# tgsstdio/BirdNest.Audio

Hardware: AMD Instinct MI355X
Metric: decoded PCM MSamples/s/GPU (bit-exact) + achieved HBM GB/s vs roofline (higher is better)
Workload: dtype int32; 1 GPU; C2: 1024-frame batches, 44.1 kHz/16-bit stereo, bs 4096, LPC-8, Rice partition order 4 -> FLACDecoder 16-bit LE interleaved PCM; frames_per_batch=1024, compressed_bytes_per_batch=10724000, pcm_bytes_per_batch=16777216, parallelism=corpus of 1 x 1024 batches partitioned per rank (shard.partition) x1

## Files before the change

birdnest/audio_amd/csrc/bnflac_kernels.hip:

```cpp
#include <hip/hip_runtime.h>
#include <stdint.h>
#include <stdlib.h>
#include <atomic>
#include <mutex>
#include <type_traits>

#include "bnflac_device.h"

#define DEV __device__ __forceinline__

__constant__ uint8_t g_crc8_tab[256];
__constant__ uint16_t g_crc16_tab[8][256];
__constant__ uint16_t g_crc16_xpow[40];
__device__ unsigned long long g_stats[16];
DEV uint64_t tnow(bool on) {
#ifndef BNFLAC_PHASE_TIMERS
    (void)on;
    return 0ull;
#endif
    if (!on) return 0ull;
    const uint64_t t = __builtin_amdgcn_s_memtime();
    asm volatile("s_waitcnt lgkmcnt(0)" ::: "memory");
    return t;
}
// ... 9 lines not shown
}
DEV u32x4 lds_ld128(const void *a) {
    u32x4 v;
    asm volatile("ds_read_b128 %0, %1" : "=v"(v) : "v"((uint32_t)(uintptr_t)a) : "memory");
    return v;
}
DEV void lds_st128(const lds_u32x4 *a, u32x4 v) {
    asm volatile("ds_write_b128 %0, %1" ::"v"((uint32_t)(uintptr_t)a), "v"(v) : "memory");
}
DEV u32x4 lds_ld128(const lds_u32x4 *a) {
    u32x4 v;
    asm volatile("ds_read_b128 %0, %1" : "=v"(v) : "v"((uint32_t)(uintptr_t)a) : "memory");
    return v;
}
DEV void lds_st64(const void *a, uint64_t v) {
    asm volatile("ds_write_b64 %0, %1" ::"v"((uint32_t)(uintptr_t)a), "v"(v) : "memory");
}
DEV uint64_t lds_ld64(const void *a) {
    uint64_t v;
    asm volatile("ds_read_b64 %0, %1" : "=v"(v) : "v"((uint32_t)(uintptr_t)a) : "memory");
    return v;
}
typedef __attribute__((address_space(1))) const void gvoid;
DEV void gst128(uint64_t addr, u32x4 v) { *(__attribute__((address_space(1))) u32x4 *)addr = v; }

#define BNF_MODE_WREDO 0x4000u
#define BNF_MODE_SW 0x8000u
#define BNF_ABLATE_NO_SW 0x10000u
#define BNF_MODE_LIST 0x20000u
#define BNF_MODE_SEG 0x80000000u
#define BNF_MODE_NOST 0x40000u
#define BNF_MODE_STREDO 0x80000u
#define BNF_ABLATE_NO_W8SPLIT 0x100000u

#define RING_MAX 16
#define RING_LANE_DW 256

struct BR {
    const uint32_t *__restrict__ w;
    uint32_t nw;
    uint32_t nblk;
    lds_u32 *ring;
    lds_u32 *lring;
    uint32_t rdepth, wmask;
    uint32_t wi, s, hi, lo, nx;
    uint32_t vendw, iend;
    uint32_t iend_old;
    uint32_t ra, vlim;
    bool stats;
};

DEV void br_init(BR &b, const uint32_t *words, uint64_t nbytes, lds_u32 *ring, uint32_t lane, uint32_t rdepth) {
    b.rdepth = rdepth;
    b.wmask = 4u * rdepth - 1u;
    b.w = words;
    b.nblk = (uint32_t)((nbytes + 15u) >> 4);
    b.nw = b.nblk * 4u;
    b.ring = ring;
    b.lring = ring + lane * 4u;
    b.wi = 2;
    b.s = b.hi = b.lo = b.nx = 0;
    b.vendw = b.iend = 0;
    b.iend_old = 0;
    b.stats = false;
}

// ... 614 lines not shown
#define CRC_LINES 4

DEV uint32_t byte_keep(int32_t lo, int32_t hi, int32_t w) {
    const int32_t a = min(max(lo - 4 * w, 0), 4), b = min(max(hi - 4 * w, 0), 4);
    const uint32_t mlo = a >= 4 ? 0u : (0xFFFFFFFFu << (8 * a));
    const uint32_t mhi = b >= 4 ? 0xFFFFFFFFu : ((1u << (8 * b)) - 1u);
    return mlo & mhi;
}
DEV bool crcz_zero(const CrcZ &c) {
    if (__builtin_popcount(c.px) & 1) return false;
    uint64_t v = ((uint64_t)(c.r1 & 0x0FFFFFFFu) << 32) | c.r0;
#pragma unroll
    for (int i = 0; i < 4; i++) {
        const uint64_t h = v >> 15;
        v = (v & 0x7FFFu) ^ h ^ (h << 1);
    }
    return v == 0;
}
DEV void crcz_line(CrcZ &c, uint4 (&v)[4], uint32_t h) {
    if (h) {
#pragma unroll
        for (int u = 0; u < 4; u++) {
            v[u].x &= st_hmask(h, 16u * u);
            v[u].y &= st_hmask(h, 16u * u + 4u);
            v[u].z &= st_hmask(h, 16u * u + 8u);
            v[u].w &= st_hmask(h, 16u * u + 12u);
        }
    }
#pragma unroll
    for (int u = 0; u < 4; u++) crcz_blk(c, v[u]);
}
template <int NL = CRC_LINES>
DEV bool st_crc16_ok(const uint8_t *__restrict__ bytes, uint64_t b0, uint64_t b1, CrcZ c = CrcZ{0u, 0u, 0u},
                     uint64_t from = 0) {
    const uint64_t p0 = max(b0 & ~(uint64_t)63u, from);
    const uint32_t h = p0 < b0 ? (uint32_t)(b0 & 63u) : 0u;
    const uint32_t nl = b1 > p0 ? (uint32_t)((b1 - p0) >> 6) : 0u;
    uint64_t p = p0;
    if (nl) {
        const uint4 *q = (const uint4 *)(bytes + p0);
        uint4 buf[NL][4];
#pragma unroll
        for (int d = 0; d < NL; d++)
#pragma unroll
            for (int u = 0; u < 4; u++) buf[d][u] = q[4u * min((uint32_t)d, nl - 1u) + u];
#pragma unroll
        for (int u = 0; u < 4; u++) {
            buf[0][u].x &= st_hmask(h, 16u * u);
            buf[0][u].y &= st_hmask(h, 16u * u + 4u);
            buf[0][u].z &= st_hmask(h, 16u * u + 8u);
            buf[0][u].w &= st_hmask(h, 16u * u + 12u);
        }
        for (uint32_t i = 0; i < nl; i += NL) {
#pragma unroll
            for (int d = 0; d < NL; d++) {
                if (i + d < nl) {
#pragma unroll
                    for (int u = 0; u < 4; u++) crcz_blk(c, buf[d][u]);
                    const uint32_t j = min(i + d + NL, nl - 1u);
#pragma unroll
                    for (int u = 0; u < 4; u++) buf[d][u] = q[4u * j + u];
                }
            }
        }
        p = p0 + (uint64_t)nl * 64u;
    }
    const uint32_t nr = (uint32_t)((b1 - p + 15u) >> 4);
    uint4 t[4];
#pragma unroll
    for (uint32_t i = 0; i < 4; i++) t[i] = i < nr ? *(const uint4 *)(bytes + p + 16u * i) : make_uint4(0u, 0u, 0u, 0u);
#pragma unroll
    for (uint32_t i = 0; i < 4; i++) {
        if (i < nr) {
            const int64_t lo = (int64_t)b0 - (int64_t)(p + 16u * i), hi = (int64_t)b1 - (int64_t)(p + 16u * i);
            const int32_t l32 = (int32_t)max(min(lo, (int64_t)16), (int64_t)0);
            const int32_t h32 = (int32_t)max(min(hi, (int64_t)16), (int64_t)0);
            uint4 v = t[i];
            v.x &= byte_keep(l32, h32, 0);
            v.y &= byte_keep(l32, h32, 1);
            v.z &= byte_keep(l32, h32, 2);
            v.w &= byte_keep(l32, h32, 3);
            crcz_blk(c, v);
        }
    }
    return crcz_zero(c);
}
#define CRCP_WORDS 8u
DEV bool st_crc16_frame(const uint8_t *__restrict__ bytes, const uint32_t *__restrict__ crcp, uint32_t f, uint64_t b0,
                        uint64_t b1) {
    if (crcp) {
        const u32x4 v = *(const u32x4 *)(crcp + CRCP_WORDS * (uint64_t)f + 4u);
        if (v.x && v.z == (uint32_t)b0 && b0 + v.x == b1) return v.y != 0u;
        const u32x4 q = *(const u32x4 *)(crcp + CRCP_WORDS * (uint64_t)f);
        const uint64_t from = ((b0 >> 6) + q.z - 1u) * 64u;
        if (q.z && q.w == (uint32_t)b0 && from <= b1)
            return st_crc16_ok(bytes, b0, b1, CrcZ{q.x, q.y & 0x0FFFFFFFu, q.y >> 31}, from);
    }
    return st_crc16_ok(bytes, b0, b1);
}

DEV uint32_t ffbh_b(uint32_t x) { return x ? (uint32_t)__builtin_clz(x) : ~0u; }

DEV uint32_t pk_ra(uint32_t wi, uint32_t lane) { return ((wi & 3u) << 2) | (lane << 4) | (((wi >> 2) & 7u) << 10); }
DEV void pk_resync(BR &b, uint32_t lane) {
    b.ra = pk_ra(b.wi, lane);
    b.vlim = b.vendw - 1u;
}
DEV void pk_next_word(BR &b) { b.nx = *(const lds_u32 *)((const __attribute__((address_space(3))) uint8_t *)b.ring + b.ra); }
DEV void pk_step(BR &b, uint32_t &rem, uint32_t k1, bool &stall, uint32_t laneb) {
    const bool live = rem != 0u;
    const uint32_t w = br_peek(b);
    const uint32_t q1 = min(ffbh_b(w), 32u);
    const uint32_t len1 = q1 + k1;
    const uint32_t q2 = ffbh_b((w << (len1 & 31u)) | 1u);
    const uint32_t len2 = len1 + q2 + k1;
    const bool fit1 = live & (len1 <= 32u);
    const bool fit2 = fit1 & (rem >= 2u) & (len2 <= 32u);
// ... 1859 lines not shown
                                                    uint64_t *__restrict__ d_offs, uint64_t *__restrict__ d_os,
                                                    bnf_frame_info *__restrict__ d_info, uint32_t cap,
                                                    uint32_t *__restrict__ nframes) {
    const uint32_t i = blockIdx.x * 256u + threadIdx.x;
    if (i >= ncand || !mark[i]) return;
    const uint32_t p = pos[i];
    if (p >= cap) return;
    const uint64_t os = out_sample[p];
    if (sp.has_stream_info && sp.total_samples > 0 && os >= sp.total_samples) {
        atomicMin(nframes, p);
        return;
    }
    d_offs[p] = cand[i];
    if (d_os) d_os[p] = os;
    if (d_info) {
        bnf_frame_info fi = info[i];
        fi.out_sample = os;
        d_info[p] = fi;
    }
}
#endif

#if BNF_TU == 3 || BNF_TU == 4 || BNF_TU == 7
#define ST_CHK 16
#define ST2_CHK 32
#define ST_RD 8

struct StCh {
    BR b;
    uint32_t cp[4];
    uint32_t q[8];
    int32_t sh;
    uint32_t k, km, k1, k32;
    uint32_t esc, left, pidx, nparts, psamples, plen, pesc, porder, order;
    uint32_t wasted;
    int32_t lim, mx, mn;
};

DEV uint32_t st_pk(int32_t lo, int32_t hi) { return __builtin_amdgcn_perm((uint32_t)hi, (uint32_t)lo, 0x05040100u); }
typedef short st_s2 __attribute__((ext_vector_type(2)));
DEV int32_t st_d2(uint32_t a, uint32_t b, int32_t acc) {
    return __builtin_amdgcn_sdot2(__builtin_bit_cast(st_s2, a), __builtin_bit_cast(st_s2, b), acc, false);
}
DEV int32_t st_d2z(uint32_t a, uint32_t b) {
    int32_t r;
    asm("v_dot2_i32_i16 %0, %1, %2, 0" : "=v"(r) : "v"(a), "v"(b));
    return r;
}

DEV bool st_setup(StCh &z, uint32_t bps, uint32_t bs, uint64_t limit) {
    SubHdr h;
    int32_t warm[8], coef[8], err = -1;
    const uint32_t st = parse_subframe_head<true, 8>(z.b, bps, bs, limit, h, warm, coef, err);
    if (st != BNF_ST_OK) return false;
    if (h.type != T_FIXED && h.type != T_LPC) return false;
    if (h.type == T_LPC && (h.order > 8 || h.path == P_WIDE)) return false;
    if (h.bps > 17) return false;
    int32_t c[8], w[8];
    bool in16 = true;
#pragma unroll
    for (int t = 0; t < 8; t++) {
        c[t] = 0;
        w[t] = ((uint32_t)t < h.order) ? warm[t] : 0;
        in16 = in16 && w[t] >= -32768 && w[t] <= 32767;
    }
    if (!in16) return false;
    z.sh = 0;
    z.lim = 0x7FFF;
    if (h.type == T_LPC) {
#pragma unroll
        for (int t = 0; t < 8; t++) c[t] = ((uint32_t)t < h.order) ? coef[t] : 0;
        if (h.path == P_MMX16) z.sh = ((uint32_t)h.shift >= 32u) ? 31 : h.shift;
        else z.sh = h.shift & 31;
    } else {
        const uint32_t o = h.order;
        c[0] = o == 1 ? 1 : o == 2 ? 2 : o == 3 ? 3 : o == 4 ? 4 : 0;
        c[1] = o == 2 ? -1 : o == 3 ? -3 : o == 4 ? -6 : 0;
        c[2] = o == 3 ? 1 : o == 4 ? 4 : 0;
        c[3] = o == 4 ? -1 : 0;
    }
#pragma unroll
    for (int k = 0; k < 4; k++) z.cp[k] = st_pk(c[2 * k], c[2 * k + 1]);
#pragma unroll
    for (int t = 0; t < 8; t++) z.q[t] = st_pk(w[t], t ? w[t - 1] : 0);
    z.order = h.order;
    z.wasted = h.wasted;
    z.porder = h.porder;
    z.nparts = 1u << h.porder;
    z.psamples = h.porder ? bs >> h.porder : bs - h.order;
    z.plen = h.rice2 ? 5u : 4u;
    z.pesc = h.rice2 ? 31u : 15u;
    z.left = 0;
    z.pidx = 0;
    z.esc = 0;
    z.k = 0;
    z.km = 31;
    z.k1 = 1;
    z.k32 = 32;
    z.mx = 0;
    z.mn = 0;
    return true;
}

template <class Z>
DEV void st_partition(Z &z) {
    const uint32_t kk = br_read(z.b, z.plen);
    z.left = (z.porder == 0 || z.pidx > 0) ? z.psamples : z.psamples - z.order;
    if (kk < z.pesc) {
        z.k = kk;
        z.esc = 0;
    } else {
        z.k = br_read(z.b, 5);
        z.esc = 1;
    }
    z.km = 31u - z.k;
    z.k1 = z.k + 1u;
    z.k32 = 32u - z.k;
    z.pidx++;
}

DEV void st_land(BR &b, uint32_t nst) {
    STAT(b.stats, 2);
    wait_vm_n(nst);
    b.vendw = b.iend * 4u;
    if (b.wi >= b.vendw) {
        br_refill(b);
        wait_vm();
// ... 16 lines not shown

template <class Z>
DEV int32_t st_rice(Z &z, uint64_t limit, uint32_t &trunc, uint32_t nst) {
    const uint32_t w = br_peek(z.b);
    const uint32_t q = ffbh(w);
    const bool slow = q >= z.k32;
    uint32_t u = (q << z.k) | __builtin_amdgcn_ubfe(w, z.km - q, z.k);
    const bool anyslow = any_lane(slow);
    st_adv(z.b, slow ? 0u : q + z.k1, nst);
    if (__builtin_expect(anyslow, 0)) {
        STAT(z.b.stats, 3);
        if (slow) {
            uint32_t qq;
            if (!br_unary(z.b, qq, limit)) trunc = 1;
            u = (qq << z.k) | br_read(z.b, z.k);
        }
    }
    return (int32_t)((u >> 1) ^ (0u - (u & 1u)));
}

template <class Z>
DEV int32_t st_next(Z &z, uint64_t limit, uint32_t &trunc, uint32_t nst) {
    while (z.left == 0) {
        if (z.pidx >= z.nparts) {
            trunc = 1;
            return 0;
        }
        st_partition(z);
    }
    z.left--;
    if (z.esc) return br_read_s(z.b, z.k);
    return st_rice(z, limit, trunc, nst);
}

template <int I>
DEV void st_dot2(const StCh &a, const StCh &b, int32_t &pa, int32_t &pb) {
#define Q_(z, j) z.q[(I + 8 - (j)) & 7]
    pa = st_d2(a.cp[3], Q_(a, 7), st_d2(a.cp[2], Q_(a, 5), st_d2(a.cp[1], Q_(a, 3), st_d2z(a.cp[0], Q_(a, 1)))));
    pb = st_d2(b.cp[3], Q_(b, 7), st_d2(b.cp[2], Q_(b, 5), st_d2(b.cp[1], Q_(b, 3), st_d2z(b.cp[0], Q_(b, 1)))));
#undef Q_
}

template <int T>
DEV void st_pre2(const StCh &a, const StCh &b, int32_t &pa, int32_t &pb) {
#define P_(z, j) z.q[(T + 8 - (j)) & 7]
    pa = st_d2(a.cp[3], P_(a, 6), st_d2(a.cp[2], P_(a, 4), st_d2z(a.cp[1], P_(a, 2))));
    pb = st_d2(b.cp[3], P_(b, 6), st_d2(b.cp[2], P_(b, 4), st_d2z(b.cp[1], P_(b, 2))));
#undef P_
}
DEV void st_fin2(const StCh &a, const StCh &b, uint32_t qa, uint32_t qb, int32_t prea, int32_t preb, int32_t &pa,
                 int32_t &pb) {
    pa = st_d2(a.cp[0], qa, prea);
    pb = st_d2(b.cp[0], qb, preb);
}

DEV void st_range(StCh &z, int32_t s0, int32_t s1) {
    z.mx = max(z.mx, max(s0, s1));
    z.mn = min(z.mn, min(s0, s1));
}

DEV void st_decor4(bool uni, uint32_t as_u, uint32_t as, int32_t (&L)[4], int32_t (&R)[4]) {
    const uint32_t a = uni ? as_u : as;
    if (a == 1) {
#pragma unroll
        for (int q = 0; q < 4; q++) R[q] = (int32_t)((uint32_t)L[q] - (uint32_t)R[q]);
    } else if (a == 2) {
// ... 84 lines not shown
        }
    }
    return true;
}

DEV uint32_t st_refill_issue(BR &b, bool want) {
    const uint32_t cg = (b.wi >> 2) & ~3u;
    const bool go = want && b.iend == cg + 4u;
    const uint32_t h = b.iend & 4u;
    const bool whole = b.iend + 3u < b.nblk;
    const uint32_t *a = b.w + (uint64_t)b.iend * 4u;
    uint32_t nd = 0;
#pragma unroll
    for (int g = 0; g < 2; g++) {
        const bool gg = go && h == 4u * (uint32_t)g;
        if (__any(gg)) {
            nd += 4u;
            if (gg) {
                lds_u32 *row = b.ring + 4u * (uint32_t)g * RING_LANE_DW;
                if (__builtin_expect(whole, 1)) {
                    lds_dma16_off<0>(a, row);
                    lds_dma16_off<16>(a, row + RING_LANE_DW);
                    lds_dma16_off<32>(a, row + 2 * RING_LANE_DW);
                    lds_dma16_off<48>(a, row + 3 * RING_LANE_DW);
                } else {
#pragma unroll
                    for (int k = 0; k < 4; k++) dma_block(b, b.iend + (uint32_t)k, 4u * (uint32_t)g + (uint32_t)k);
                }
            }
        }
    }
    if (go) b.iend += 4u;
    return nd;
}


DEV uint32_t st_ra(uint32_t wi, uint32_t lane) { return ((wi & 3u) << 2) | (lane << 4) | (((wi >> 2) & 7u) << 10); }
DEV void st_adv_nc(BR &b, uint32_t n, uint32_t laneb) {
    uint32_t t;
    const bool c = __builtin_usub_overflow(b.s, n, &t);
    b.s = t & 31u;
    b.hi = c ? b.lo : b.hi;
    b.lo = c ? __builtin_bswap32(b.nx) : b.lo;
    b.wi += (uint32_t)c;
    b.ra = (((b.ra | 0x3F3u) + (uint32_t)c) & 0x1C0Cu) | laneb;
}
DEV void st_next_word(BR &b) { b.nx = *(const lds_u32 *)((const __attribute__((address_space(3))) uint8_t *)b.ring + b.ra); }
DEV void st_resync(BR &b, uint32_t lane) {
    b.ra = st_ra(b.wi, lane);
    b.vlim = b.vendw - 1u;
}
template <class Z>
DEV void st_rare(Z &z, bool sl, bool ld, uint32_t &u, uint64_t limit, uint32_t &trunc, uint32_t nst,
                uint32_t lane) {
    if (any_lane(ld)) {
        st_land(z.b, nst);
        if (z.b.wi + 1u >= z.b.vendw) {
            wait_vm();
            br_refill(z.b);
            wait_vm();
            br_drained(z.b);
        }
        st_next_word(z.b);
    }
    if (any_lane(sl)) {
        STAT(z.b.stats, 3);
// ... 30 lines not shown
    switch (i) {
    case 0: lo = st_qperm<0x00>(lo); hi = st_qperm<0x00>(hi); break;
    case 1: lo = st_qperm<0x55>(lo); hi = st_qperm<0x55>(hi); break;
    case 2: lo = st_qperm<0xAA>(lo); hi = st_qperm<0xAA>(hi); break;
    default: lo = st_qperm<0xFF>(lo); hi = st_qperm<0xFF>(hi); break;
    }
    return ((uint64_t)hi << 32) | lo;
}

template <int T, int FMT, int AS, int PO, int NPK>
DEV void st_lpc_out(StCh &z0, StCh &z1, uint32_t u0, uint32_t u1, int32_t (&L)[4], int32_t (&R)[4], bool as_uni,
                    uint32_t as_u, uint32_t as, uint8_t *dst, uint32_t nbase, bool al, uint32_t bs, bool store,
                    u32x4 (&pk)[NPK], int32_t &pre0, int32_t &pre1, bool anyw) {
    constexpr bool STG = (FMT == BNF_OUT_FLACDECODER || FMT == BNF_OUT_FILEREADER);
    int32_t p0, p1, n0, n1;
    st_fin2(z0, z1, z0.q[(T + 7) & 7], z1.q[(T + 7) & 7], pre0, pre1, p0, p1);
    st_pre2<T>(z0, z1, n0, n1);
    pre0 = n0;
    pre1 = n1;
    const int32_t s0 = (int32_t)(((u0 >> 1) ^ (0u - (u0 & 1u))) + (uint32_t)(p0 >> z0.sh));
    const int32_t s1 = (int32_t)(((u1 >> 1) ^ (0u - (u1 & 1u))) + (uint32_t)(p1 >> z1.sh));
    if (T & 1) {
        st_range(z0, L[(T + 3) & 3], s0);
        st_range(z1, R[(T + 3) & 3], s1);
    }
    z0.q[T] = __builtin_amdgcn_perm(z0.q[(T + 7) & 7], (uint32_t)s0, 0x05040100u);
    z1.q[T] = __builtin_amdgcn_perm(z1.q[(T + 7) & 7], (uint32_t)s1, 0x05040100u);
    L[T & 3] = s0;
    R[T & 3] = s1;
    if ((T & 3) == 3) {
        if (AS < 0 && __builtin_expect(anyw, 0)) {
#pragma unroll
            for (int q = 0; q < 4; q++) {
                L[q] = (int32_t)((uint32_t)L[q] << z0.wasted);
                R[q] = (int32_t)((uint32_t)R[q] << z1.wasted);
            }
        }
        if (STG && AS >= 0) {
            pk[PO + (T >> 2)] = st_pack4<AS>(z0.q[(T + 6) & 7], z1.q[(T + 6) & 7], z0.q[T], z1.q[T]);
            return;
        }
        st_decor4t<AS>(as_uni, as_u, as, L, R);
        if (STG) {
            uint32_t w[4];
#pragma unroll
            for (int q = 0; q < 4; q++) w[q] = __builtin_amdgcn_perm((uint32_t)R[q], (uint32_t)L[q], 0x05040100u);
            pk[PO + (T >> 2)] = u32x4{w[0], w[1], w[2], w[3]};
        } else if (store) {
            st_emit4<FMT>(dst, nbase + (uint32_t)T - 3u, 4u, al, bs, L, R);
        }
    }
}

DEV uint32_t st_rice_pair(const StCh &z, uint32_t &ua, uint32_t &ub, bool &sl) {
    const uint32_t w = br_peek(z.b);
    const uint32_t qa = (uint32_t)__builtin_clz(w | 1u);
    const uint32_t la = qa + z.k1;
    const uint32_t w2 = w << (la & 31u);
    const uint32_t qb = (uint32_t)__builtin_clz(w2 | 1u);
    ua = (qa << z.k) | __builtin_amdgcn_ubfe(w, z.km - qa, z.k);
    ub = (qb << z.k) | __builtin_amdgcn_ubfe(w2, z.km - qb, z.k);
    const uint32_t n = la + qb + z.k1;
    sl = n > 32u;
    return sl ? 0u : n;
}
DEV void st_rare_pair(StCh &z, bool sl, bool ld, uint32_t &ua, uint32_t &ub, uint64_t limit, uint32_t &trunc,
                      uint32_t nst, uint32_t lane) {
    if (any_lane(ld)) {
// ... 24 lines not shown
                       uint32_t bs, bool store, u32x4 (&pk)[NPK], int32_t &pre0, int32_t &pre1,
                       uint32_t lane, bool anyw) {
    static_assert((T & 1) == 0, "pairs start on even samples");
    constexpr bool STG = (FMT == BNF_OUT_FLACDECODER || FMT == BNF_OUT_FILEREADER);
    constexpr uint32_t spg = (FMT == BNF_OUT_INTERLEAVED32 || FMT == BNF_OUT_PLANAR32) ? 2u : 1u;
    const uint32_t nqt = nq + ((!STG && T >= 4 && store) ? spg : 0u);
    uint32_t u0a, u0b, u1a, u1b;
    bool sl0, sl1;
    const uint32_t n0 = st_rice_pair(z0, u0a, u0b, sl0), n1 = st_rice_pair(z1, u1a, u1b, sl1);
    const uint32_t laneb = lane << 4;
    st_adv_nc(z0.b, n0, laneb);
    st_adv_nc(z1.b, n1, laneb);
    constexpr bool CHK = (T & 2) == 0;
    const bool ld0 = CHK && z0.b.wi >= z0.b.vlim, ld1 = CHK && z1.b.wi >= z1.b.vlim;
    st_next_word(z0.b);
    st_next_word(z1.b);
    if (__builtin_expect(any_lane(sl0 || sl1 || ld0 || ld1), 0)) {
        st_rare_pair(z0, sl0, ld0, u0a, u0b, limit, trunc, nqt, lane);
        st_rare_pair(z1, sl1, ld1, u1a, u1b, limit, trunc, nqt, lane);
    }
    st_lpc_out<T, FMT, AS, PO, NPK>(z0, z1, u0a, u1a, L, R, as_uni, as_u, as, dst, nbase, al, bs, store, pk, pre0, pre1, anyw);
    st_lpc_out<T + 1, FMT, AS, PO, NPK>(z0, z1, u0b, u1b, L, R, as_uni, as_u, as, dst, nbase, al, bs, store, pk, pre0, pre1, anyw);
}

template <int T, int FMT>
DEV bool st_gen_step(StCh &z0, StCh &z1, int32_t (&L)[4], int32_t (&R)[4], uint64_t limit, uint32_t &trunc,
                     uint32_t nst, bool as_uni, uint32_t as_u, uint32_t as, uint8_t *dst, uint32_t n, bool valid,
                     bool al, uint32_t bs, bool store) {
    const bool v = valid && n < bs;
    int32_t s0 = 0, s1 = 0;
    if (v) {
        int32_t p0, p1;
        st_dot2<T>(z0, z1, p0, p1);
        if (n < z0.order) s0 = (int32_t)(int16_t)z0.q[T];
        else s0 = (int32_t)((uint32_t)st_next(z0, limit, trunc, nst) + (uint32_t)(p0 >> z0.sh));
        if (n < z1.order) s1 = (int32_t)(int16_t)z1.q[T];
        else s1 = (int32_t)((uint32_t)st_next(z1, limit, trunc, nst) + (uint32_t)(p1 >> z1.sh));
        st_range(z0, s0, s0);
        st_range(z1, s1, s1);
        z0.q[T] = __builtin_amdgcn_perm(z0.q[(T + 7) & 7], (uint32_t)s0, 0x05040100u);
        z1.q[T] = __builtin_amdgcn_perm(z1.q[(T + 7) & 7], (uint32_t)s1, 0x05040100u);
    }
    L[T & 3] = (int32_t)((uint32_t)s0 << z0.wasted);
    R[T & 3] = (int32_t)((uint32_t)s1 << z1.wasted);
    bool stored = false;
    if ((T & 3) == 3) {
        const uint32_t nq = n - 3u;
        const uint32_t nv = (valid && nq < bs) ? min(4u, bs - nq) : 0u;
        st_decor4(as_uni, as_u, as, L, R);
        if (store) stored = st_emit4<FMT>(dst, nq, nv, al, bs, L, R);
    }
    return stored;
}

template <int FMT>
__global__ void __launch_bounds__(64, 2) k_decode_st(const uint32_t *__restrict__ words, uint64_t nbytes,
                                                     uint32_t nframes, bnf_stream_params sp, uint32_t chn_lanes,
                                                     uint8_t *__restrict__ out, uint64_t out_bytes,
                                                     bnf_frame_info *__restrict__ info,
                                                     const uint32_t *__restrict__ perm, uint32_t ablate,
                                                     const uint32_t *__restrict__ crcp) {
    constexpr bool STG = (FMT == BNF_OUT_FLACDECODER || FMT == BNF_OUT_FILEREADER);
    constexpr uint32_t ST_SPG = (FMT == BNF_OUT_INTERLEAVED32 || FMT == BNF_OUT_PLANAR32) ? 2u : 1u;
    __shared__ LDS_DMA_ALIGN uint32_t ring[2 * ST_RD * RING_LANE_DW + 1024];
    static_assert((ST_RD * RING_LANE_DW * 4) % 1024 == 0, "channel 1's ring base must stay 1 KiB aligned (LDS-DMA)");
    const uint32_t lane = threadIdx.x;
    const uint32_t slot = blockIdx.x * 64u + lane;
    const uint32_t f = (perm && slot < nframes) ? perm[slot] : slot;
    const uint64_t limit = nbytes * 8u;
    bnf_frame_info fi;
    const bool have = f < nframes;
    if (have) fi = info[f];
    const bool mine = have && fi.status == BNF_ST_OK && (fi.flags & BNF_FL_ST) && !(fi.flags & BNF_FL_REDO) &&
                      (!(ablate & BNF_MODE_WREDO) || (fi.flags & BNF_FL_WAVE_REDO));
    if (!__any(mine)) return;

    uint64_t stride = 0;
    bool ok = mine && fi.channels == 2 && chn_lanes >= 2;
    if (FMT == BNF_OUT_FLACDECODER) { stride = 4; ok = ok && fi.bps == 16 && sp.channels >= 2; }
    else if (FMT == BNF_OUT_FILEREADER) { stride = 4; ok = ok && sp.channels == 2 && sp.bps == 16; }
    else if (FMT == BNF_OUT_INTERLEAVED32) { stride = 8; ok = ok && sp.channels == 2; }
    else { stride = 4ull * sp.channels; ok = ok && sp.channels == 2; }
    const uint32_t bs = ok ? fi.blocksize : 0u;
    const uint64_t os = ok ? fi.out_sample : 0u;
    ok = ok && (os + bs) * stride <= out_bytes;
    uint8_t *dst = out + os * stride;
    const bool al = (((uintptr_t)dst) & 15u) == 0 && (FMT != BNF_OUT_PLANAR32 || (bs & 3u) == 0);

    StCh z0, z1;
    lds_u32 *ring0 = (lds_u32 *)ring, *ring1 = (lds_u32 *)ring + ST_RD * RING_LANE_DW;
    br_init(z0.b, words, nbytes, ring0, lane, ST_RD);
    br_init(z1.b, words, nbytes, ring1, lane, ST_RD);
    z0.b.stats = z1.b.stats = (ablate & 0x100u) != 0;
    STAT(z0.b.stats, 5);
    const bool tmon = z0.b.stats;
    const uint64_t t_start = tnow(tmon);
    uint64_t tm_dec = 0, tm_ref = 0, tm_pack = 0;
    if (ok) {
        br_seek(z0.b, fi.frame_off * 8u + fi.sub_start[0]);
        ok = st_setup(z0, sub_bps(fi, 0), bs, limit);
    }
    if (ok) {
        br_seek(z1.b, fi.frame_off * 8u + fi.sub_start[1]);
        ok = st_setup(z1, sub_bps(fi, 1), bs, limit);
    }
    const uint32_t as = ok ? fi.assignment : 0u;
    const bool anyw = any_lane(ok && (z0.wasted | z1.wasted) != 0u);
    const uint32_t as_u = __builtin_amdgcn_readfirstlane(as);
    const bool as_uni = !any_lane(ok && as != as_u);
    const int as_fix = (as_uni && !anyw && as_u <= 3u) ? (int)as_u : -1;
    lds_u32x4 *stg = (lds_u32x4 *)((lds_u32 *)ring + 2u * ST_RD * RING_LANE_DW);
    static_assert(sizeof(ring) >= (2 * ST_RD * RING_LANE_DW + 1024) * 4, "the flush's 4 KB staging tile lies past the two rings");

    uint32_t mybs = ok ? bs : 0u;
    for (int o = 32; o > 0; o >>= 1) mybs = max(mybs, (uint32_t)__shfl_xor(mybs, o));
    const uint32_t nchunks = (mybs + ST2_CHK - 1) / ST2_CHK;
    uint32_t trunc = 0;
    wait_vm();
    uint32_t nst = 0;
    const bool sto = !(ablate & 2u);
    auto refill = [&](bool want) {
        wait_vm_n(nst);
        z0.b.vendw = z0.b.iend * 4u;
        z1.b.vendw = z1.b.iend * 4u;
        st_refill_issue(z0.b, want);
        st_refill_issue(z1.b, want);
        nst = 0;
    };
    const uint64_t t_loop = tnow(tmon);
    for (uint32_t kc = 0; kc < nchunks; kc++) {
        const uint64_t ta = tnow(tmon);
        const uint32_t n0 = kc * ST2_CHK;
        const bool valid = ok && n0 < bs;
        bool fast = valid && n0 >= 8u && n0 + ST2_CHK <= bs && !(ablate & 12u);
        if (fast) {
            if (z0.left == 0 && z0.pidx < z0.nparts) st_partition(z0);
            if (z1.left == 0 && z1.pidx < z1.nparts) st_partition(z1);
            fast = !z0.esc && !z1.esc && z0.left >= ST2_CHK && z1.left >= ST2_CHK;
        }
        const bool fused = !any_lane(valid && !fast);
        u32x4 pk[4], pk0[4];
        if (fused) {
            if (valid) {
                STAT(z0.b.stats, 0);
                int32_t pre0, pre1;
                st_pre2<7>(z0, z1, pre0, pre1);
                st_resync(z0.b, lane);
                st_resync(z1.b, lane);
                auto chunk = [&](auto as_c) {
                    constexpr int AS = decltype(as_c)::value;
                    auto group = [&](auto g_c, uint32_t nb) {
                        constexpr uint32_t G = decltype(g_c)::value;
                        int32_t L[4], R[4];
                        const uint32_t nq = nst + (STG ? 0u : G * 2u * ST_SPG);
#define FPAIR(T) st_fused_pair<T, FMT, AS, 2 * G, 4>(z0, z1, L, R, limit, trunc, nq, as_uni, as_u, as, dst, nb, al, bs, sto, pk, pre0, pre1, lane, anyw)
                        FPAIR(0); FPAIR(2); FPAIR(4); FPAIR(6);
#undef FPAIR
                    };
#pragma unroll 1
                    for (uint32_t h = 0; h < 2; h++) {
                        const uint32_t nb = n0 + 16u * h;
                        group(std::integral_constant<uint32_t, 0>(), nb);
                        group(std::integral_constant<uint32_t, 1>(), nb + 8u);
                        if (h == 0) {
                            if (STG) {
#pragma unroll
                                for (int u = 0; u < 4; u++) pk0[u] = pk[u];
                            } else if (sto) {
                                nst += 4u * ST_SPG;
                            }
                            refill(true);
// ... 5 lines not shown
                switch (as_fix) {
                case 0: chunk(std::integral_constant<int, 0>()); break;
                case 1: chunk(std::integral_constant<int, 1>()); break;
                case 2: chunk(std::integral_constant<int, 2>()); break;
                case 3: chunk(std::integral_constant<int, 3>()); break;
                default: chunk(std::integral_constant<int, -1>()); break;
                }
                z0.left -= ST2_CHK;
                z1.left -= ST2_CHK;
            } else {
                refill(false);
            }
            if (!STG && sto && any_lane(valid)) nst += 4u * ST_SPG;
        } else {
            STAT(z0.b.stats, 1);
#pragma unroll 1
            for (uint32_t g = 0; g < ST2_CHK / 8; g++) {
                int32_t L[4], R[4];
                const uint32_t nb = n0 + g * 8u;
                bool st0, st1;
#define GSTEP(T) st_gen_step<T, FMT>(z0, z1, L, R, limit, trunc, nst, as_uni, as_u, as, dst, nb + T, valid, al, bs, sto)
                GSTEP(0); GSTEP(1); GSTEP(2);
                st0 = GSTEP(3);
                if (any_lane(st0)) nst += 1u;
                GSTEP(4); GSTEP(5); GSTEP(6);
                st1 = GSTEP(7);
                if (any_lane(st1)) nst += 1u;
#undef GSTEP
                if (g == 1) refill(valid && nb + 8u < bs);
            }
        }
        const uint64_t tb = tnow(tmon);
        tm_dec += tb - ta;
        refill(valid && n0 + ST2_CHK < bs);
        const uint64_t tc = tnow(tmon);
        tm_ref += tc - tb;
        if (STG && fused) {
            uint64_t run = (valid && sto) ? (uint64_t)(uintptr_t)(dst + (uint64_t)n0 * 4u) : 0ull;
            if ((ablate & 0x10000000u) && run && out_bytes >= (1u << 20))
                run = (uint64_t)(uintptr_t)(out + (uint64_t)(blockIdx.x & 7u) * 65536u + lane * 1024u + ((n0 * 4u) & 1023u));
            const uint32_t rlo = (uint32_t)run, rhi = (uint32_t)(run >> 32);
            const uint32_t fr = lane & 31u, ul = lane & 7u;
#pragma unroll
            for (uint32_t r = 0; r < 2; r++) {
                if ((lane >> 5) == r) {
#pragma unroll
                    for (uint32_t u = 0; u < 8; u++) lds_st128(stg + fr * 8u + (u ^ (fr & 7u)), u < 4 ? pk0[u] : pk[u - 4]);
                }
                lds_sync();
                u32x4 v[4];
                uint64_t a[4];
#pragma unroll
                for (uint32_t i = 0; i < 4; i++) {
                    const uint32_t f = (lane >> 3) + 8u * i;
                    v[i] = lds_ld128(stg + f * 8u + (ul ^ (f & 7u)));
                    const uint32_t src = (32u * r + f) * 4u;
                    a[i] = ((uint64_t)(uint32_t)__builtin_amdgcn_ds_bpermute((int)src, (int)rhi) << 32) |
                           (uint32_t)__builtin_amdgcn_ds_bpermute((int)src, (int)rlo);
                }
                lds_sync();
#pragma unroll
                for (uint32_t i = 0; i < 4; i++) {
                    if (a[i]) gst128(a[i] + 16u * ul, v[i]);
                    if (any_lane(a[i] != 0)) nst += 1u;
                }
            }
        }
        tm_pack += tnow(tmon) - tc;
    }
    const uint64_t t_loopend = tnow(tmon);

    uint32_t crc_read = 0;
    uint64_t end_byte = 0, resume = 0;
    if (ok) {
        if (z0.mx > z0.lim || z0.mn < -z0.lim - 1 || z1.mx > z1.lim || z1.mn < -z1.lim - 1) ok = false;
        if (trunc) ok = false;
    }
    if (ok) {
        while (z1.pidx < z1.nparts) {
            const uint32_t kk = br_read(z1.b, z1.plen);
            if (kk >= z1.pesc) br_read(z1.b, 5);
            z1.pidx++;
        }
        const uint32_t padbits = (uint32_t)((8u - (br_pos(z1.b) & 7u)) & 7u);
        const uint32_t zp = br_read(z1.b, padbits);
        if (br_pos(z1.b) > limit || zp != 0) ok = false;
        end_byte = br_pos(z1.b) >> 3;
        crc_read = br_read(z1.b, 16);
        if (br_pos(z1.b) > limit) ok = false;
        resume = br_pos(z1.b);
    }
    uint32_t crc = crc_read;
    if (ok && !(ablate & 1u) && !st_crc16_frame((const uint8_t *)words, crcp, f, fi.frame_off, end_byte + 2u)) ok = false;
    if (ok && crc != crc_read) ok = false;
    if (ok) {
        info[f].resume_bit = resume;
        info[f].crc16_read = crc_read;
        info[f].crc16_calc = crc;
        info[f].crc_ok = 1u;
    } else if (mine) {
        info[f].flags = fi.flags | BNF_FL_REDO;
    }
    if (tmon && lane == 0) {
        const uint64_t t_end = tnow(tmon);
        atomicAdd(&g_stats[8], (unsigned long long)(t_loop - t_start));
        atomicAdd(&g_stats[9], (unsigned long long)tm_dec);
        atomicAdd(&g_stats[10], (unsigned long long)tm_ref);
        atomicAdd(&g_stats[11], (unsigned long long)tm_pack);
        atomicAdd(&g_stats[12], (unsigned long long)(t_end - t_loopend));
    }
}

#if BNF_TU == 7
#define SW_TAPS 12
struct StW {
    BR b;
    int32_t c[SW_TAPS];
    int32_t x[16];
    int32_t sh;
    uint32_t wide;
    uint32_t k, km, k1, k32;
    uint32_t esc, left, pidx, nparts, psamples, plen, pesc, porder, order;
    uint32_t wasted;
};

DEV bool sw_setup(StW &z, uint32_t bps, uint32_t bs, uint64_t limit) {
    SubHdr h;
    int32_t warm[SW_TAPS], coef[SW_TAPS], err = -1;
    const uint32_t st = parse_subframe_head<true, SW_TAPS>(z.b, bps, bs, limit, h, warm, coef, err);
    if (st != BNF_ST_OK) return false;
    if (h.type != T_FIXED && h.type != T_LPC) return false;
    if (h.order > SW_TAPS) return false;
    if (h.type == T_LPC && h.path == P_MMX16) return false;
    if (h.type == T_LPC && h.path == P_WIDE && ((uint32_t)h.shift & 0xFFu) >= 32u) return false;
// ... 1081 lines not shown
```

birdnest/audio_amd/csrc/bnflac_runtime.cpp:

```cpp
#include <hip/hip_runtime.h>

#include <algorithm>
#include <cstdio>
#include <cstdlib>
#include <cstring>
#include <mutex>
#include <string>
#include <sys/stat.h>
#include <vector>

#include "../../../include/bnflac.h"
#include "bnflac_device.h"
#include "bnflac_md5.h"

static_assert(sizeof(bnflac_frame_info) == sizeof(bnf_frame_info), "frame info layout");
static_assert(sizeof(bnf_frame_info) == 128, "frame info is 128 bytes");
static_assert(offsetof(FLAC__FrameHeader, number) == 24, "FrameHeader.FrameOrSampleNumber @24 (LibFLACSharp.cs:232)");
static_assert(offsetof(FLAC__FrameHeader, crc) == 32, "FrameHeader.Crc @32 (LibFLACSharp.cs:233)");
static_assert(offsetof(FLAC__StreamMetadata, data) == 16, "StreamMetadata.data @16 (LibFLACSharp.cs:299)");
static_assert(offsetof(FLAC__StreamMetadata, data.stream_info.sample_rate) == 32, "sample_rate @32");
static_assert(offsetof(FLAC__StreamMetadata, data.stream_info.total_samples) == 48, "total_samples @48");

extern "C" {
hipError_t bnf_upload_tables(const uint8_t *crc8, const uint16_t *crc16x8, const uint16_t *xpow);
// ... 56 lines not shown

struct DevGuard {
    int prev = -1;
    explicit DevGuard(int dev) {
        if (hipGetDevice(&prev) != hipSuccess) prev = -1;
        if (prev != dev) (void)hipSetDevice(dev);
    }
    ~DevGuard() {
        int cur = -1;
        if (prev >= 0 && hipGetDevice(&cur) == hipSuccess && cur != prev) (void)hipSetDevice(prev);
    }
};

static std::mutex g_dev_mu;
static bool g_tables_ready[64];

static int ensure_device(int dev) {
    int n = 0;
    if (hipGetDeviceCount(&n) != hipSuccess || n <= 0) return fail("bnflac: no HIP device available (the decode path is GPU-only)");
    if (dev < 0 || dev >= n || dev >= 64) return fail("bnflac: bad device index");
    std::lock_guard<std::mutex> lk(g_dev_mu);
    DevGuard g(dev);
    if (!g_tables_ready[dev]) {
        uint8_t c8[256];
        uint16_t c16[8 * 256], xp[40];
        build_tables(c8, c16, xp);
        if (bnf_upload_tables(c8, c16, xp) != hipSuccess) return fail("bnflac: table upload failed");
        g_tables_ready[dev] = true;
    }
    return 0;
}

extern "C" BNFLAC_API void bnflac_debug_set_ablate(uint32_t flags) { bnf_set_ablate(flags); }
extern "C" void bnf_set_parse_wave(int mode);
extern "C" BNFLAC_API void bnflac_debug_set_parse_wave(int mode) { bnf_set_parse_wave(mode); }
extern "C" void bnf_set_decode_sys(int mode);
extern "C" BNFLAC_API void bnflac_debug_set_decode_sys(int mode) { bnf_set_decode_sys(mode); }
extern "C" int bnf_crc_mode();
extern "C" void bnf_set_crc_mode(int mode);
extern "C" BNFLAC_API void bnflac_debug_set_crc_mode(int mode) { bnf_set_crc_mode(mode); }
extern "C" uint64_t bnf_decode_seg_launches();
extern "C" BNFLAC_API uint64_t bnflac_debug_decode_seg_launches(void) { return bnf_decode_seg_launches(); }
extern "C" hipError_t bnf_parse_wave_stats(uint64_t *out8, int reset);
extern "C" BNFLAC_API int bnflac_debug_parse_wave_stats(uint64_t *out8, int reset) {
    return bnf_parse_wave_stats(out8, reset) == hipSuccess ? 0 : -1;
}
extern "C" BNFLAC_API int bnflac_debug_stats(uint64_t *out16, int reset) {
    return bnf_stats(out16, reset) == hipSuccess ? 0 : fail("bnflac_debug_stats failed");
}

extern "C" BNFLAC_API int bnflac_device_count(void) {
    int n = 0;
    if (hipGetDeviceCount(&n) != hipSuccess) return 0;
    return n;
}

struct CtxBuf {
    void *p = nullptr;
    size_t cap = 0;
    bool grow(size_t n) {
        if (n <= cap) return true;
        if (p) (void)hipFree(p);
        p = nullptr;
        cap = 0;
        if (hipMalloc(&p, n) != hipSuccess) return false;
        cap = n;
// ... 1213 lines not shown
```

include/bnflac.h:

```cpp
#ifndef BNFLAC_H
#define BNFLAC_H

#include "FLAC_compat.h"

#ifdef __cplusplus
extern "C" {
#endif

#if defined(__GNUC__)
#define BNFLAC_API __attribute__((visibility("default")))
#else
#define BNFLAC_API
#endif


BNFLAC_API FLAC__StreamDecoder *FLAC__stream_decoder_new(void);
BNFLAC_API FLAC__bool FLAC__stream_decoder_finish(FLAC__StreamDecoder *decoder);
BNFLAC_API FLAC__bool FLAC__stream_decoder_delete(FLAC__StreamDecoder *decoder);
BNFLAC_API int FLAC__stream_decoder_init_file(FLAC__StreamDecoder *decoder, const char *filename,
                                              FLAC__StreamDecoderWriteCallback write_callback,
                                              FLAC__StreamDecoderMetadataCallback metadata_callback,
                                              FLAC__StreamDecoderErrorCallback error_callback,
                                              void *client_data);
BNFLAC_API FLAC__bool FLAC__stream_decoder_process_single(FLAC__StreamDecoder *decoder);
// ... 51 lines not shown
    BNFLAC_OUT_FLACDECODER = 2,
    BNFLAC_OUT_FILEREADER = 3
};

typedef struct bnflac_ctx bnflac_ctx;

BNFLAC_API int bnflac_ctx_create(int device, bnflac_ctx **out);
BNFLAC_API void bnflac_ctx_destroy(bnflac_ctx *ctx);
BNFLAC_API const char *bnflac_last_error(void);
BNFLAC_API int bnflac_device_count(void);

BNFLAC_API int bnflac_index_frames(bnflac_ctx *ctx, const uint8_t *d_bytes, uint64_t nbytes,
                                   uint64_t *d_offsets, uint32_t cap, uint32_t *d_count, void *hip_stream);

BNFLAC_API int bnflac_index_stream(bnflac_ctx *ctx, const uint8_t *d_bytes, uint64_t nbytes, uint64_t first_offset,
                                   const bnflac_stream_params *sp, uint64_t *d_frame_offsets, uint64_t *d_out_sample,
                                   bnflac_frame_info *d_info, uint32_t cap, uint32_t *d_nframes, void *hip_stream);

BNFLAC_API int bnflac_decode_frames(bnflac_ctx *ctx, const uint8_t *d_bytes, uint64_t nbytes,
                                    const uint64_t *d_frame_offsets, uint32_t nframes,
                                    const bnflac_stream_params *sp, const uint64_t *d_out_sample,
                                    uint64_t base_sample, int out_format, uint8_t *d_out, uint64_t out_bytes,
                                    bnflac_frame_info *d_info, void *hip_stream);

BNFLAC_API int bnflac_parse_frames(bnflac_ctx *ctx, const uint8_t *d_bytes, uint64_t nbytes,
                                   const uint64_t *d_frame_offsets, uint32_t nframes,
                                   const bnflac_stream_params *sp, const uint64_t *d_out_sample,
                                   uint64_t base_sample, bnflac_frame_info *d_info, void *hip_stream);
BNFLAC_API int bnflac_decode_parsed(bnflac_ctx *ctx, const uint8_t *d_bytes, uint64_t nbytes, uint32_t nframes,
                                    const bnflac_stream_params *sp, int out_format, uint8_t *d_out,
                                    uint64_t out_bytes, bnflac_frame_info *d_info, void *hip_stream);

BNFLAC_API void bnflac_debug_set_ablate(uint32_t flags);
BNFLAC_API void bnflac_debug_set_parse_wave(int mode);
BNFLAC_API void bnflac_debug_set_decode_sys(int mode);
BNFLAC_API void bnflac_debug_set_crc_mode(int mode);
BNFLAC_API int bnflac_debug_crc_handoff(bnflac_ctx *ctx, uint32_t *out, uint32_t nframes);
BNFLAC_API uint64_t bnflac_debug_decode_seg_launches(void);
BNFLAC_API int bnflac_debug_parse_wave_stats(uint64_t *out8, int reset);
BNFLAC_API int bnflac_debug_stats(uint64_t *out16, int reset);

BNFLAC_API uint32_t bnflac_out_stride(int out_format, const bnflac_stream_params *sp);

BNFLAC_API int bnflac_md5_interleaved32(const int32_t *pcm, uint64_t nsamples, uint32_t channels, uint32_t bps,
                                        uint8_t out_md5[16]);


typedef struct bnflac_reader bnflac_reader;
BNFLAC_API int bnflac_reader_open(int device, const uint8_t *bytes, uint64_t nbytes, int out_format,
                                  uint32_t window_frames, bnflac_reader **out);
BNFLAC_API int bnflac_reader_params(const bnflac_reader *reader, bnflac_stream_params *sp, uint64_t *total_bytes,
                                    uint32_t *nframes);
BNFLAC_API int64_t bnflac_reader_read(bnflac_reader *reader, uint8_t *buf, uint64_t count);
BNFLAC_API int bnflac_reader_seek(bnflac_reader *reader, uint64_t sample);
BNFLAC_API int64_t bnflac_reader_read_filereader(bnflac_reader *reader, uint8_t *buffer, uint64_t offset,
                                                 uint64_t num_bytes, uint64_t buffer_length);
BNFLAC_API void bnflac_reader_close(bnflac_reader *reader);
BNFLAC_API int bnflac_reader_pool_release(int device);
BNFLAC_API const char *bnflac_reader_last_error(void);

#ifdef __cplusplus
}
#endif

#endif
```

Measured before the change: 726,800 MSamples/s.

## Fold frame CRC16 over LDS ring lines during stereo decode refills

Computes the frame CRC16 incrementally from the bit-reader's LDS ring buffer while refilling during subframe decode, seeded from the per-frame CRC prefix table. The final CRC check then resumes from the folded state and skips re-reading most of the frame from global memory. Per-channel subframe state is also packed into one bitfield word to cut register pressure. This adds LDS reads and wave-divergent loops inside the refill path and more complex bookkeeping for where the fold stopped.

```diff
diff --git a/birdnest/audio_amd/csrc/bnflac_kernels.hip b/birdnest/audio_amd/csrc/bnflac_kernels.hip
--- a/birdnest/audio_amd/csrc/bnflac_kernels.hip
+++ b/birdnest/audio_amd/csrc/bnflac_kernels.hip
@@ -65,6 +65,7 @@
 #define BNF_MODE_NOST 0x40000u
 #define BNF_MODE_STREDO 0x80000u
 #define BNF_ABLATE_NO_W8SPLIT 0x100000u
+#define BNF_ABLATE_NO_STFOLD 0x40u
 
 #define RING_MAX 16
 #define RING_LANE_DW 256
@@ -745,7 +746,7 @@
 }
 template <int NL = CRC_LINES>
 DEV bool st_crc16_ok(const uint8_t *__restrict__ bytes, uint64_t b0, uint64_t b1, CrcZ c = CrcZ{0u, 0u, 0u},
-                     uint64_t from = 0) {
+                     uint64_t from = 0, CrcZ *fin = nullptr) {
     const uint64_t p0 = max(b0 & ~(uint64_t)63u, from);
     const uint32_t h = p0 < b0 ? (uint32_t)(b0 & 63u) : 0u;
     const uint32_t nl = b1 > p0 ? (uint32_t)((b1 - p0) >> 6) : 0u;
@@ -796,6 +797,7 @@
             crcz_blk(c, v);
         }
     }
+    if (fin) *fin = c;
     return crcz_zero(c);
 }
 #define CRCP_WORDS 8u
@@ -2721,10 +2723,19 @@
     uint32_t q[8];
     int32_t sh;
     uint32_t k, km, k1, k32;
-    uint32_t esc, left, pidx, nparts, psamples, plen, pesc, porder, order;
-    uint32_t wasted;
-    int32_t lim, mx, mn;
+    uint32_t left;
+    uint32_t pw;
+    int32_t mx, mn;
+    DEV uint32_t pidx() const { return pw & 0xFFFFu; }
+    DEV uint32_t porder() const { return (pw >> 16) & 15u; }
+    DEV uint32_t order() const { return (pw >> 20) & 15u; }
+    DEV uint32_t plen() const { return 4u + ((pw >> 24) & 1u); }
+    DEV uint32_t pesc() const { return (pw & (1u << 24)) ? 31u : 15u; }
+    DEV uint32_t wasted() const { return (pw >> 25) & 31u; }
+    DEV bool esc() const { return (pw & (1u << 30)) != 0u; }
+    DEV bool parts_left() const { return pidx() < (1u << porder()); }
 };
+#define ST_LIM 0x7FFF
 
 DEV uint32_t st_pk(int32_t lo, int32_t hi) { return __builtin_amdgcn_perm((uint32_t)hi, (uint32_t)lo, 0x05040100u); }
 typedef short st_s2 __attribute__((ext_vector_type(2)));
@@ -2755,7 +2766,6 @@
     }
     if (!in16) return false;
     z.sh = 0;
-    z.lim = 0x7FFF;
     if (h.type == T_LPC) {
 #pragma unroll
         for (int t = 0; t < 8; t++) c[t] = ((uint32_t)t < h.order) ? coef[t] : 0;
@@ -2772,16 +2782,8 @@
     for (int k = 0; k < 4; k++) z.cp[k] = st_pk(c[2 * k], c[2 * k + 1]);
 #pragma unroll
     for (int t = 0; t < 8; t++) z.q[t] = st_pk(w[t], t ? w[t - 1] : 0);
-    z.order = h.order;
-    z.wasted = h.wasted;
-    z.porder = h.porder;
-    z.nparts = 1u << h.porder;
-    z.psamples = h.porder ? bs >> h.porder : bs - h.order;
-    z.plen = h.rice2 ? 5u : 4u;
-    z.pesc = h.rice2 ? 31u : 15u;
+    z.pw = ((h.porder & 15u) << 16) | ((h.order & 15u) << 20) | ((h.rice2 ? 1u : 0u) << 24) | ((h.wasted & 31u) << 25);
     z.left = 0;
-    z.pidx = 0;
-    z.esc = 0;
     z.k = 0;
     z.km = 31;
     z.k1 = 1;
@@ -2864,6 +2866,34 @@
     if (z.esc) return br_read_s(z.b, z.k);
     return st_rice(z, limit, trunc, nst);
 }
+DEV void st_partition(StCh &z, uint32_t bs) {
+    const uint32_t kk = br_read(z.b, z.plen());
+    const uint32_t po = z.porder(), ps = po ? bs >> po : bs - z.order();
+    z.left = (po == 0 || z.pidx() > 0) ? ps : ps - z.order();
+    if (kk < z.pesc()) {
+        z.k = kk;
+        z.pw &= ~(1u << 30);
+    } else {
+        z.k = br_read(z.b, 5);
+        z.pw |= 1u << 30;
+    }
+    z.km = 31u - z.k;
+    z.k1 = z.k + 1u;
+    z.k32 = 32u - z.k;
+    z.pw++;
+}
+DEV int32_t st_next(StCh &z, uint32_t bs, uint64_t limit, uint32_t &trunc, uint32_t nst) {
+    while (z.left == 0) {
+        if (!z.parts_left()) {
+            trunc = 1;
+            return 0;
+        }
+        st_partition(z, bs);
+    }
+    z.left--;
+    if (z.esc()) return br_read_s(z.b, z.k);
+    return st_rice(z, limit, trunc, nst);
+}
 
 template <int I>
 DEV void st_dot2(const StCh &a, const StCh &b, int32_t &pa, int32_t &pb) {
@@ -3014,6 +3044,80 @@
     }
     if (go) b.iend += 4u;
     return nd;
+}
+
+struct StFold {
+    CrcZ c;
+    uint32_t fl;
+};
+DEV void st_fold_point(StFold &r, const BR &b, uint32_t lane, bool want, bool end, bool ahead) {
+    const uint32_t cl = b.wi >> 4, il = b.iend >> 2;
+    const uint32_t lim = cl + ((end && ahead) ? 1u : 0u);
+#pragma unroll 1
+    for (;;) {
+        const bool go = want && r.fl < lim && r.fl < il && (end ? r.fl + 2u >= il : (r.fl + 2u == il && il == cl + 1u));
+        if (!any_lane(go)) break;
+        if (go) {
+            const lds_u32x4 *p = (const lds_u32x4 *)(b.ring + (r.fl & 1u) * (4u * RING_LANE_DW) + lane * 4u);
+            u32x4 a = lds_ld128(p), c = lds_ld128(p + RING_LANE_DW / 4u);
+            asm volatile("s_waitcnt lgkmcnt(0)" : "+v"(a), "+v"(c)::"memory");
+            crcz_blk(r.c, make_uint4(a.x, a.y, a.z, a.w));
+            a = lds_ld128(p + 2u * (RING_LANE_DW / 4u));
+            crcz_blk(r.c, make_uint4(c.x, c.y, c.z, c.w));
+            c = lds_ld128(p + 3u * (RING_LANE_DW / 4u));
+            asm volatile("s_waitcnt lgkmcnt(0)" : "+v"(a), "+v"(c)::"memory");
+            crcz_blk(r.c, make_uint4(a.x, a.y, a.z, a.w));
+            crcz_blk(r.c, make_uint4(c.x, c.y, c.z, c.w));
+            r.fl++;
+        }
+    }
+}
+DEV void st_fold_start(StFold &r, const BR &b, const uint32_t *__restrict__ words, const uint32_t *__restrict__ crcp,
+                       uint32_t f, uint64_t frame_off, bool on) {
+    r.c = CrcZ{0u, 0u, 0u};
+    r.fl = ~0u;
+    if (on) {
+        const u32x4 q = *(const u32x4 *)(crcp + CRCP_WORDS * (uint64_t)f);
+        if (q.z && q.w == (uint32_t)frame_off) {
+            r.c = CrcZ{q.x, q.y & 0x0FFFFFFFu, q.y >> 31};
+            r.fl = (uint32_t)(frame_off >> 6) + q.z - 1u;
+        }
+    }
+    const bool behind = r.fl != ~0u && r.fl + 3u == (b.iend >> 2);
+    if (any_lane(behind)) {
+        if (behind) {
+            const uint4 *g = (const uint4 *)((const uint8_t *)words + (uint64_t)r.fl * 64u);
+            uint4 v[4];
+#pragma unroll
+            for (uint32_t i = 0; i < 4; i++) v[i] = g[i];
+            crcz_line(r.c, v, 0u);
+            r.fl++;
+        }
+    }
+}
+DEV bool st_crc16_run(const uint8_t *__restrict__ bytes, const uint32_t *__restrict__ crcp, uint32_t f, uint64_t b0,
+                      uint64_t b1, const StFold &r, bool &used, CrcZ *fin = nullptr) {
+    CrcZ c = CrcZ{0u, 0u, 0u};
+    uint64_t from = 0;
+    used = false;
+    if (crcp) {
+        const u32x4 v = *(const u32x4 *)(crcp + CRCP_WORDS * (uint64_t)f + 4u);
+        if (v.x && v.z == (uint32_t)b0 && b0 + v.x == b1) return v.y != 0u;
+    }
+    const uint64_t rf = (uint64_t)r.fl * 64u;
+    if (r.fl != ~0u && rf <= b1 && rf > b0) {
+        c = r.c;
+        from = rf;
+        used = true;
+    } else if (crcp) {
+        const u32x4 q = *(const u32x4 *)(crcp + CRCP_WORDS * (uint64_t)f);
+        const uint64_t pf = ((b0 >> 6) + q.z - 1u) * 64u;
+        if (q.z && q.w == (uint32_t)b0 && pf <= b1) {
+            c = CrcZ{q.x, q.y & 0x0FFFFFFFu, q.y >> 31};
+            from = pf;
+        }
+    }
+    return st_crc16_ok(bytes, b0, b1, c, from, fin);
 }
 
 
@@ -3110,8 +3214,8 @@
         if (AS < 0 && __builtin_expect(anyw, 0)) {
 #pragma unroll
             for (int q = 0; q < 4; q++) {
-                L[q] = (int32_t)((uint32_t)L[q] << z0.wasted);
-                R[q] = (int32_t)((uint32_t)R[q] << z1.wasted);
+                L[q] = (int32_t)((uint32_t)L[q] << z0.wasted());
+                R[q] = (int32_t)((uint32_t)R[q] << z1.wasted());
             }
         }
         if (STG && AS >= 0) {
@@ -3202,17 +3306,17 @@
     if (v) {
         int32_t p0, p1;
         st_dot2<T>(z0, z1, p0, p1);
-        if (n < z0.order) s0 = (int32_t)(int16_t)z0.q[T];
-        else s0 = (int32_t)((uint32_t)st_next(z0, limit, trunc, nst) + (uint32_t)(p0 >> z0.sh));
-        if (n < z1.order) s1 = (int32_t)(int16_t)z1.q[T];
-        else s1 = (int32_t)((uint32_t)st_next(z1, limit, trunc, nst) + (uint32_t)(p1 >> z1.sh));
+        if (n < z0.order()) s0 = (int32_t)(int16_t)z0.q[T];
+        else s0 = (int32_t)((uint32_t)st_next(z0, bs, limit, trunc, nst) + (uint32_t)(p0 >> z0.sh));
+        if (n < z1.order()) s1 = (int32_t)(int16_t)z1.q[T];
+        else s1 = (int32_t)((uint32_t)st_next(z1, bs, limit, trunc, nst) + (uint32_t)(p1 >> z1.sh));
         st_range(z0, s0, s0);
         st_range(z1, s1, s1);
         z0.q[T] = __builtin_amdgcn_perm(z0.q[(T + 7) & 7], (uint32_t)s0, 0x05040100u);
         z1.q[T] = __builtin_amdgcn_perm(z1.q[(T + 7) & 7], (uint32_t)s1, 0x05040100u);
     }
-    L[T & 3] = (int32_t)((uint32_t)s0 << z0.wasted);
-    R[T & 3] = (int32_t)((uint32_t)s1 << z1.wasted);
+    L[T & 3] = (int32_t)((uint32_t)s0 << z0.wasted());
+    R[T & 3] = (int32_t)((uint32_t)s1 << z1.wasted());
     bool stored = false;
     if ((T & 3) == 3) {
         const uint32_t nq = n - 3u;
@@ -3275,7 +3379,7 @@
         ok = st_setup(z1, sub_bps(fi, 1), bs, limit);
     }
     const uint32_t as = ok ? fi.assignment : 0u;
-    const bool anyw = any_lane(ok && (z0.wasted | z1.wasted) != 0u);
+    const bool anyw = any_lane(ok && (z0.wasted() | z1.wasted()) != 0u);
     const uint32_t as_u = __builtin_amdgcn_readfirstlane(as);
     const bool as_uni = !any_lane(ok && as != as_u);
     const int as_fix = (as_uni && !anyw && as_u <= 3u) ? (int)as_u : -1;
@@ -3286,14 +3390,18 @@
     for (int o = 32; o > 0; o >>= 1) mybs = max(mybs, (uint32_t)__shfl_xor(mybs, o));
     const uint32_t nchunks = (mybs + ST2_CHK - 1) / ST2_CHK;
     uint32_t trunc = 0;
+    const bool fold_on = crcp != nullptr && !(ablate & (BNF_ABLATE_NO_STFOLD | 1u));
+    StFold fold;
+    st_fold_start(fold, z1.b, words, crcp, f, ok ? fi.frame_off : 0u, fold_on && ok);
     wait_vm();
     uint32_t nst = 0;
     const bool sto = !(ablate & 2u);
-    auto refill = [&](bool want) {
+    auto refill = [&](bool want, bool end = false, bool ahead = false) {
         wait_vm_n(nst);
         z0.b.vendw = z0.b.iend * 4u;
         z1.b.vendw = z1.b.iend * 4u;
         st_refill_issue(z0.b, want);
+        if (fold_on) st_fold_point(fold, z1.b, lane, want, end, ahead);
         st_refill_issue(z1.b, want);
         nst = 0;
     };
@@ -3304,9 +3412,9 @@
         const bool valid = ok && n0 < bs;
         bool fast = valid && n0 >= 8u && n0 + ST2_CHK <= bs && !(ablate & 12u);
         if (fast) {
-            if (z0.left == 0 && z0.pidx < z0.nparts) st_partition(z0);
-            if (z1.left == 0 && z1.pidx < z1.nparts) st_partition(z1);
-            fast = !z0.esc && !z1.esc && z0.left >= ST2_CHK && z1.left >= ST2_CHK;
+            if (z0.left == 0 && z0.parts_left()) st_partition(z0, bs);
+            if (z1.left == 0 && z1.parts_left()) st_partition(z1, bs);
+            fast = !z0.esc() && !z1.esc() && z0.left >= ST2_CHK && z1.left >= ST2_CHK;
         }
         const bool fused = !any_lane(valid && !fast);
         u32x4 pk[4], pk0[4];
@@ -3378,7 +3486,8 @@
         }
         const uint64_t tb = tnow(tmon);
         tm_dec += tb - ta;
-        refill(valid && n0 + ST2_CHK < bs);
+        const uint32_t rest = bs - min(bs, n0 + ST2_CHK), inp = z1.esc() ? 0u : min(rest, z1.left);
+        refill(valid && n0 + ST2_CHK < bs, true, inp * z1.k1 + (rest - inp) >= 576u);
         const uint64_t tc = tnow(tmon);
         tm_ref += tc - tb;
         if (STG && fused) {
@@ -3419,14 +3528,14 @@
     uint32_t crc_read = 0;
     uint64_t end_byte = 0, resume = 0;
     if (ok) {
-        if (z0.mx > z0.lim || z0.mn < -z0.lim - 1 || z1.mx > z1.lim || z1.mn < -z1.lim - 1) ok = false;
+        if (z0.mx > ST_LIM || z0.mn < -ST_LIM - 1 || z1.mx > ST_LIM || z1.mn < -ST_LIM - 1) ok = false;
         if (trunc) ok = false;
     }
     if (ok) {
-        while (z1.pidx < z1.nparts) {
-            const uint32_t kk = br_read(z1.b, z1.plen);
-            if (kk >= z1.pesc) br_read(z1.b, 5);
-            z1.pidx++;
+        while (z1.parts_left()) {
+            const uint32_t kk = br_read(z1.b, z1.plen());
+            if (kk >= z1.pesc()) br_read(z1.b, 5);
+            z1.pw++;
         }
         const uint32_t padbits = (uint32_t)((8u - (br_pos(z1.b) & 7u)) & 7u);
         const uint32_t zp = br_read(z1.b, padbits);
@@ -3436,8 +3545,28 @@
         if (br_pos(z1.b) > limit) ok = false;
         resume = br_pos(z1.b);
     }
+    const uint32_t fl_flags = mine ? info[f].flags : 0u;
+    const uint64_t frame_off = ok ? info[f].frame_off : 0u;
     uint32_t crc = crc_read;
-    if (ok && !(ablate & 1u) && !st_crc16_frame((const uint8_t *)words, crcp, f, fi.frame_off, end_byte + 2u)) ok = false;
+    if (ok && !(ablate & 1u)) {
+        bool used;
+#ifdef BNFLAC_CRC_FOLD_CHECK
+        CrcZ ra = CrcZ{0u, 0u, 0u}, rb = CrcZ{0u, 0u, 0u};
+        StFold none;
+        none.c = CrcZ{0u, 0u, 0u};
+        none.fl = ~0u;
+        bool unused;
+        const bool va = st_crc16_run((const uint8_t *)words, crcp, f, frame_off, end_byte + 2u, fold, used, &ra);
+        const bool vb = st_crc16_run((const uint8_t *)words, crcp, f, frame_off, end_byte + 2u, none, unused, &rb);
+        const bool differ = used && (va != vb || ra.r0 != rb.r0 || ((ra.r1 ^ rb.r1) & 0x0FFFFFFFu) != 0u ||
+                                     (__builtin_popcount(ra.px ^ rb.px) & 1) != 0);
+        if (differ) atomicAdd(&g_stats[7], 1ull);
+        if (!va) ok = false;
+#else
+        if (!st_crc16_run((const uint8_t *)words, crcp, f, frame_off, end_byte + 2u, fold, used)) ok = false;
+#endif
+        if (z0.b.stats && used) atomicAdd(&g_stats[6], 1ull);
+    }
     if (ok && crc != crc_read) ok = false;
     if (ok) {
         info[f].resume_bit = resume;
@@ -3445,7 +3574,7 @@
         info[f].crc16_calc = crc;
         info[f].crc_ok = 1u;
     } else if (mine) {
-        info[f].flags = fi.flags | BNF_FL_REDO;
+        info[f].flags = fl_flags | BNF_FL_REDO;
     }
     if (tmon && lane == 0) {
         const uint64_t t_end = tnow(tmon);
diff --git a/birdnest/audio_amd/csrc/bnflac_runtime.cpp b/birdnest/audio_amd/csrc/bnflac_runtime.cpp
--- a/birdnest/audio_amd/csrc/bnflac_runtime.cpp
+++ b/birdnest/audio_amd/csrc/bnflac_runtime.cpp
@@ -112,6 +112,13 @@
 }
 
 extern "C" BNFLAC_API void bnflac_debug_set_ablate(uint32_t flags) { bnf_set_ablate(flags); }
+extern "C" BNFLAC_API int bnflac_debug_crc_fold_check(void) {
+#ifdef BNFLAC_CRC_FOLD_CHECK
+    return 1;
+#else
+    return 0;
+#endif
+}
 extern "C" void bnf_set_parse_wave(int mode);
 extern "C" BNFLAC_API void bnflac_debug_set_parse_wave(int mode) { bnf_set_parse_wave(mode); }
 extern "C" void bnf_set_decode_sys(int mode);
diff --git a/include/bnflac.h b/include/bnflac.h
--- a/include/bnflac.h
+++ b/include/bnflac.h
@@ -107,6 +107,7 @@
                                     uint64_t out_bytes, bnflac_frame_info *d_info, void *hip_stream);
 
 BNFLAC_API void bnflac_debug_set_ablate(uint32_t flags);
+BNFLAC_API int bnflac_debug_crc_fold_check(void);
 BNFLAC_API void bnflac_debug_set_parse_wave(int mode);
 BNFLAC_API void bnflac_debug_set_decode_sys(int mode);
 BNFLAC_API void bnflac_debug_set_crc_mode(int mode);
```

Measured after the change: 744,500 MSamples/s (median of 6 runs). 2.4% higher.
